# bywmm/RE-GNN

Measured on NVIDIA B200. Metric: GTEPS fwd+bwd per RE-layer, higher is better.
Workload: dtype f32

## Files before the change

re_gnn_b200/csrc/spmm.cu:

```cuda
#include <initializer_list>

#include "common.cuh"

namespace regnn {

struct SpmmArgs {
  const int32_t* indptr;
  const int32_t* indices;
  const uint8_t* etype;
  const float* theta;
  float alpha;
  int R;
  const float* norm_src;
  const float* norm_dst;
  const float* X;
  int64_t ldx;
  float* Y;
  int64_t ldy;
  int64_t row_begin, row_end;
  int F;
  const int32_t* frag_row;
  const int32_t* frag_begin;
  int nfrag, nfrag_pad, threshold;
  float* partial;
// ... 508 lines not shown
    const int64_t vi = wi * GPW + grp;
    int64_t v = -1;
    int begin = 0, len = 0;
    const bool is_frag = vi < a.nfrag;
    if (vi < nitems) {
      if (is_frag) {
        v = a.frag_row[vi];
        begin = a.frag_begin[vi];
        len = min(a.threshold, a.indptr[v + 1] - begin);
      } else {
        v = sa.order[vi - a.nfrag];
        begin = a.indptr[v];
        len = a.indptr[v + 1] - begin;
      }
    }
    const int maxlen = __reduce_max_sync(0xffffffffu, len);
    const float nd = (v >= 0 && a.norm_dst != nullptr) ? a.norm_dst[v] : 1.f;
    float4 trow = make_float4(0.f, 0.f, 0.f, 0.f);
    if (BINS && v >= 0 && col_ok) trow = ldg4(sa.Xrow + (size_t)v * sa.ldr + lg * 4);
    const bool want_ydg = DNORM && (sa.dn_sides & 2) && v >= 0 && col_ok && !is_frag;
    if constexpr (DNORM) {
      if (want_ydg) {
        prefetch_l2(sa.Yfwd + (size_t)v * sa.ldyf + lg * 4);
        prefetch_l2(xbytes + (uint64_t)(uint32_t)v * ldxb);
      }
    }
    float4 acc = make_float4(0.f, 0.f, 0.f, 0.f);
    int cur_rel = 0;
    float racc = 0.f;
    const int32_t* ip = a.indices + begin;
    const uint8_t* ep = a.etype + begin;

    if constexpr (kCoop) {
      static_assert(G % U == 0, "a round must not straddle a slot batch");
      const int gbase = lane & ~(G - 1);
      auto load_batch = [&](int t0, int& bi, int& be, float& bn) {
        const int t = t0 + lg;
        bi = -1;
        be = 0;
        bn = 0.f;
        if (t < len) {
          bi = __ldg(ip + t);
          be = weighted ? (int)__ldg(ep + t) : 0;
          bn = a.norm_src != nullptr ? __ldg(a.norm_src + bi) : 1.f;
        }
      };
      int nbi, nbe;
      float nbn;
      load_batch(0, nbi, nbe, nbn);
      for (int t0 = 0; t0 < maxlen; t0 += G) {
        const int bi = nbi, be = nbe;
        const float bn = nbn;
        const float bc = (weighted ? w_s[be] : 1.f) * bn;
        if (t0 + G < maxlen) load_batch(t0 + G, nbi, nbe, nbn);
        const int cnt = min(G, maxlen - t0);
        for (int j = 0; j < cnt; j += U) {
          float4 x[U];
#pragma unroll
          for (int u = 0; u < U; ++u) {
            const int si = __shfl_sync(0xffffffffu, bi, gbase + j + u);
            x[u] = si >= 0 ? ldg4(reinterpret_cast<const float*>(xbytes + (uint64_t)(uint32_t)si * ldxb))
                           : make_float4(0.f, 0.f, 0.f, 0.f);
          }
#pragma unroll
          for (int u = 0; u < U; ++u) {
            const int from = gbase + j + u;
            fma4(acc, __shfl_sync(0xffffffffu, bc, from), x[u]);
            if (BINS) {
              const int se = __shfl_sync(0xffffffffu, be, from);
              const float sn = __shfl_sync(0xffffffffu, bn, from);
              const float d = dot4(x[u], trow);
              if (t0 + j + u < len && se != cur_rel) {
                mybins[cur_rel * 32] += racc;
                racc = 0.f;
                cur_rel = se;
              }
              racc = fmaf(sn * nd, d, racc);
            }
          }
        }
      }
    } else {
      int nidx[U], net[U];
#pragma unroll
      for (int u = 0; u < U; ++u) {
        nidx[u] = u < len ? __ldg(ip + u) : -1;
        net[u] = (weighted && u < len) ? (int)__ldg(ep + u) : 0;
      }
      for (int t = 0; t < maxlen; t += U) {
        int idx[U], et[U];
#pragma unroll
        for (int u = 0; u < U; ++u) {
          idx[u] = nidx[u];
          et[u] = net[u];
        }
        float4 x[U];
        float ns[U];
#pragma unroll
        for (int u = 0; u < U; ++u) {
          x[u] = idx[u] >= 0 ? ldg4(reinterpret_cast<const float*>(xbytes + (uint64_t)(uint32_t)idx[u] * ldxb))
                             : make_float4(0.f, 0.f, 0.f, 0.f);
          ns[u] = idx[u] >= 0 ? (a.norm_src != nullptr ? __ldg(a.norm_src + idx[u]) : 1.f) : 0.f;
        }
#pragma unroll
        for (int u = 0; u < U; ++u) {
          const int tn = t + U + u;
          nidx[u] = tn < len ? __ldg(ip + tn) : -1;
          net[u] = (weighted && tn < len) ? (int)__ldg(ep + tn) : 0;
        }
#pragma unroll
        for (int u = 0; u < U; ++u) {
          const float coef = (weighted ? w_s[et[u]] : 1.f) * ns[u];
          fma4(acc, coef, x[u]);
          if (BINS) {
            const float d = dot4(x[u], trow);
            if (idx[u] >= 0 && et[u] != cur_rel) {
              mybins[cur_rel * 32] += racc;
              racc = 0.f;
              cur_rel = et[u];
            }
            racc = fmaf(ns[u] * nd, d, racc);
          }
        }
      }
    }
    if (BINS) {
      mybins[cur_rel * 32] += racc;
      if constexpr (DNORM) {
        float p = (sa.dn_sides & 1) ? dot4(acc, trow) * nd : 0.f;
        if (want_ydg)
          p += dot4(ldg4(sa.Yfwd + (size_t)v * sa.ldyf + lg * 4),
                    ldg4(reinterpret_cast<const float*>(xbytes + (uint64_t)(uint32_t)v * ldxb)));
        p = group_sum<G>(p);
        if (lg == 0 && v >= 0 && !is_frag) sa.d_norm[v] = p / sa.norm[v];
      } else if (sa.xdx != nullptr) {
        const float d = group_sum<G>(dot4(acc, trow)) * nd;
        if (lg == 0 && v >= 0 && !is_frag) sa.xdx[v] = d;
      }
    }
    if (v >= 0 && col_ok) {
      if (is_frag) {
        st4(a.partial + (size_t)vi * a.F + lg * 4, acc);
      } else {
        scale4(acc, nd);
        float* yrow = sa.peers.base != nullptr ? sa.peers.row(v) : a.Y + (size_t)v * a.ldy;
        st4(yrow + lg * 4, acc);
        if (!BINS && sa.peers.base != nullptr && sa.Ylocal != nullptr) st4(sa.Ylocal + (size_t)v * sa.ldl + lg * 4, acc);
      }
    }
  }
  if (BINS) reduce_bins(bins, scratch, a.R, sa.partials + (size_t)blockIdx.x * a.R);
}

constexpr int kRowdotRows = 4;
__global__ void __launch_bounds__(kWarpsPerBlock * 32)
rowdot_norm_kernel(const float* __restrict__ norm, int sides, const float* __restrict__ X, int64_t ldx,
                   const float* __restrict__ Y, int64_t ldy, const float* __restrict__ G, int64_t ldg,
                   const float* __restrict__ dX, int64_t lddx, const float* __restrict__ xdx, int F,
                   int64_t row_begin, int64_t row_end, float* __restrict__ d_norm) {
  const int lane = threadIdx.x & 31;
  const int64_t v0 = row_begin + ((int64_t)blockIdx.x * kWarpsPerBlock + (threadIdx.x >> 5)) * kRowdotRows;
  if (v0 >= row_end) return;
  const bool use_x = (sides & 1) && xdx == nullptr;
  const bool vec = (F & 3) == 0 && ((ldy | ldg) & 3) == 0 && ((((uintptr_t)Y) | ((uintptr_t)G)) & 15) == 0 &&
                   (!use_x || (((ldx | lddx) & 3) == 0 && ((((uintptr_t)X) | ((uintptr_t)dX)) & 15) == 0));
  float p[kRowdotRows];
#pragma unroll
  for (int r = 0; r < kRowdotRows; ++r) p[r] = 0.f;
  if (vec) {
    for (int c = lane * 4; c < F; c += 128) {
#pragma unroll
      for (int r = 0; r < kRowdotRows; ++r) {
        const int64_t v = v0 + r;
        if (v < row_end) {
          if (sides & 2) p[r] += dot4(ldg4(Y + (size_t)v * ldy + c), ldg4(G + (size_t)v * ldg + c));
          if (use_x) p[r] += dot4(ldg4(X + (size_t)v * ldx + c), ldg4(dX + (size_t)v * lddx + c));
        }
      }
    }
  } else {
    for (int c = lane; c < F; c += 32) {
#pragma unroll
      for (int r = 0; r < kRowdotRows; ++r) {
        const int64_t v = v0 + r;
        if (v < row_end) {
          if (sides & 2) p[r] = fmaf(__ldg(Y + (size_t)v * ldy + c), __ldg(G + (size_t)v * ldg + c), p[r]);
          if (use_x) p[r] = fmaf(__ldg(X + (size_t)v * ldx + c), __ldg(dX + (size_t)v * lddx + c), p[r]);
        }
      }
    }
  }
#pragma unroll
  for (int r = 0; r < kRowdotRows; ++r) {
    const int64_t v = v0 + r;
    float t = group_sum<32>(p[r]);
    if (v < row_end && lane == 0) {
      if ((sides & 1) && xdx != nullptr) t += xdx[v];
      d_norm[v] = t / norm[v];
    }
  }
}

__global__ void long_row_dnorm_kernel(const int32_t* __restrict__ long_rows, int num_long, const float* __restrict__ X,
                                      int64_t ldx, const float* __restrict__ dX, int64_t lddx, int F, int64_t row_begin,
                                      int64_t row_end, float* __restrict__ xdx, const float* __restrict__ Y, int64_t ldy,
                                      const float* __restrict__ Gd, int64_t ldg, const float* __restrict__ norm, int sides,
                                      float* __restrict__ d_norm) {
  const int lane = threadIdx.x & 31;
  const int l = blockIdx.x * (blockDim.x >> 5) + (threadIdx.x >> 5);
  if (l >= num_long) return;
  const int64_t v = long_rows[l];
  if (v < row_begin || v >= row_end) return;
  float p = 0.f, q = 0.f;
  if (xdx != nullptr || (sides & 1))
    for (int c = lane; c < F; c += 32) p = fmaf(__ldg(X + (size_t)v * ldx + c), dX[(size_t)v * lddx + c], p);
  if (d_norm != nullptr && (sides & 2))
    for (int c = lane; c < F; c += 32) q = fmaf(__ldg(Y + (size_t)v * ldy + c), __ldg(Gd + (size_t)v * ldg + c), q);
  p = group_sum<32>(p);
  q = group_sum<32>(q);
  if (lane == 0) {
    if (xdx != nullptr) xdx[v] = p;
    if (d_norm != nullptr) d_norm[v] = (((sides & 1) ? p : 0.f) + q) / norm[v];
  }
}

struct SpmmBwdArgs {
  const int32_t* indptr;
  const int32_t* indices;
  const uint8_t* etype;
  int R;
  const float* norm;
  int sides;
  const float* X;  int64_t ldx;
  const float* Y;  int64_t ldy;
  const float* G;  int64_t ldg;
  const float* dX; int64_t lddx;
  int64_t row_begin, row_end;
  int F;
  double* partials;
  float* d_norm;
  const int32_t* frag_row;
  const int32_t* frag_begin;
  int nfrag, threshold;
};

template <int G, int C, int VW, bool WEIGHTED>
__global__ void __launch_bounds__(kWarpsPerBlock * 32)
spmm_bwd_w_kernel(SpmmBwdArgs a) {
  using V = Vec<VW>;
  using T = typename V::T;
  constexpr int U = Unroll<C>::U;
  constexpr int GPW = 32 / G;
  extern __shared__ __align__(16) unsigned char smem_raw[];
  double* scratch = reinterpret_cast<double*>(smem_raw);
  float* bins = reinterpret_cast<float*>(scratch + kWarpsPerBlock * a.R);
  const int lane = threadIdx.x & 31, warp = threadIdx.x >> 5;
  const int lg = lane % G, grp = lane / G;
  float* mybins = bins + (size_t)warp * a.R * 32 + lane;
  if (WEIGHTED)
    for (int r = 0; r < a.R; ++r) mybins[r * 32] = 0.f;

  bool col_ok[C];
#pragma unroll
  for (int k = 0; k < C; ++k) col_ok[k] = (lg + k * G) * VW < a.F;
  const int64_t rows = a.row_end - a.row_begin;
  const int64_t nfrag_groups = (a.nfrag + GPW - 1) / GPW;
  const int64_t ngroups = nfrag_groups + (rows + GPW - 1) / GPW;

  for (int64_t rg = (int64_t)blockIdx.x * kWarpsPerBlock + warp; rg < ngroups;
       rg += (int64_t)gridDim.x * kWarpsPerBlock) {
    bool row_ok = false, first = true;
    int64_t v = 0;
    int s0 = 0, len = 0;
    if (rg < nfrag_groups) {
      const int64_t fi = rg * GPW + grp;
      if (fi < a.nfrag) {
        v = a.frag_row[fi];
        if (v >= a.row_begin && v < a.row_end) {
          s0 = a.frag_begin[fi];
          len = min(a.threshold, a.indptr[v + 1] - s0);
          first = s0 == a.indptr[v];
          row_ok = true;
        }
      }
    } else {
      v = a.row_begin + (rg - nfrag_groups) * GPW + grp;
      if (v < a.row_end) {
        s0 = a.indptr[v];
        len = a.indptr[v + 1] - s0;
        row_ok = len <= a.threshold;
        if (!row_ok) len = 0;
      }
    }
    float nv = 1.f;
    T g[C];
    float p = 0.f;
    if (row_ok) nv = a.norm != nullptr ? a.norm[v] : 1.f;
#pragma unroll
    for (int k = 0; k < C; ++k) {
      g[k] = V::zero();
      if (row_ok && col_ok[k]) {
        const size_t c = (size_t)(lg + k * G) * VW;
        g[k] = V::load(a.G + (size_t)v * a.ldg + c);
        if (first && a.d_norm != nullptr) {
          if (a.sides & 2) p += V::dot(V::load(a.Y + (size_t)v * a.ldy + c), g[k]);
          if (a.sides & 1) p += V::dot(V::load(a.X + (size_t)v * a.ldx + c), V::load(a.dX + (size_t)v * a.lddx + c));
// ... 281 lines not shown

#define REGNN_DISPATCH_GC(G_, C_, VW_, CALL)                    \
  if (sh.G == G_ && sh.C == C_ && sh.VW == VW_) {               \
    constexpr int G = G_, C = C_, VW = VW_;                     \
    CALL;                                                       \
    launched = true;                                            \
  }
#define REGNN_DISPATCH_SHAPES(CALL)                                                            \
  REGNN_DISPATCH_GC(4, 1, 4, CALL) REGNN_DISPATCH_GC(8, 1, 4, CALL) REGNN_DISPATCH_GC(16, 1, 4, CALL) \
  REGNN_DISPATCH_GC(16, 2, 4, CALL) REGNN_DISPATCH_GC(16, 3, 4, CALL)                          \
  REGNN_DISPATCH_GC(32, 1, 4, CALL) REGNN_DISPATCH_GC(32, 2, 4, CALL) REGNN_DISPATCH_GC(32, 3, 4, CALL) \
  REGNN_DISPATCH_GC(32, 4, 4, CALL) REGNN_DISPATCH_GC(32, 8, 4, CALL)                          \
  REGNN_DISPATCH_GC(4, 1, 1, CALL) REGNN_DISPATCH_GC(8, 1, 1, CALL) REGNN_DISPATCH_GC(16, 1, 1, CALL) \
  REGNN_DISPATCH_GC(32, 1, 1, CALL) REGNN_DISPATCH_GC(32, 2, 1, CALL) REGNN_DISPATCH_GC(32, 3, 1, CALL) \
  REGNN_DISPATCH_GC(32, 4, 1, CALL) REGNN_DISPATCH_GC(32, 8, 1, CALL)

}

using namespace regnn;

extern "C" int regnn_relation_counts(const int32_t* row, const uint8_t* etype_csr, int64_t num_edges,
                                     int64_t num_nodes, int num_relations, int32_t* counts, void* stream) {
  REGNN_REQUIRE(counts && (num_edges == 0 || (row && etype_csr)), REGNN_ERR_INVALID_ARG, "relation_counts: null pointer");
  REGNN_REQUIRE(num_relations >= 1 && num_relations <= REGNN_MAX_RELATIONS, REGNN_ERR_UNSUPPORTED_SHAPE,
                "num_relations=%d outside [1,%d]", num_relations, REGNN_MAX_RELATIONS);
  cudaMemsetAsync(counts, 0, (size_t)num_nodes * num_relations * sizeof(int32_t), (cudaStream_t)stream);
  if (num_edges > 0)
    relation_count_kernel<<<(unsigned)((num_edges + 255) / 256), 256, 0, (cudaStream_t)stream>>>(row, etype_csr, num_edges,
                                                                                               num_relations, counts);
  return check_launch("regnn_relation_counts");
}

extern "C" int regnn_wdeg_norm_fwd(const int32_t* indptr, const uint8_t* etype_csr, const int32_t* counts,
                                   const float* theta, float alpha, int num_relations,
                                   float exponent, float clamp_min, int64_t row_begin, int64_t row_end, float* deg,
                                   float* norm, void* stream) {
  REGNN_REQUIRE(theta && norm && (counts || (indptr && etype_csr)), REGNN_ERR_INVALID_ARG, "wdeg_norm_fwd: null pointer");
  REGNN_REQUIRE(num_relations >= 1 && num_relations <= REGNN_MAX_RELATIONS, REGNN_ERR_UNSUPPORTED_SHAPE,
                "num_relations=%d outside [1,%d]", num_relations, REGNN_MAX_RELATIONS);
  const int64_t rows = row_end - row_begin;
  REGNN_REQUIRE(rows >= 0, REGNN_ERR_INVALID_ARG, "wdeg_norm_fwd: empty/negative row range");
  if (rows == 0) return REGNN_OK;
  const int threads = kWarpsPerBlock * 32;
  if (counts != nullptr) {
    wdeg_norm_fwd_cnt_kernel<<<(unsigned)((rows + threads - 1) / threads), threads, 0, (cudaStream_t)stream>>>(
        counts, theta, alpha, num_relations, exponent, clamp_min, row_begin, row_end, deg, norm);
  } else if (num_relations <= 32) {
    const int64_t blocks = (rows + kWarpsPerBlock * kWdegRows - 1) / (kWarpsPerBlock * kWdegRows);
    wdeg_norm_fwd_slot_kernel<<<(unsigned)blocks, threads, 0, (cudaStream_t)stream>>>(
        indptr, etype_csr, theta, alpha, num_relations, exponent, clamp_min, row_begin, row_end, deg, norm);
  } else {
    const int64_t blocks = (rows * 8 + threads - 1) / threads;
    wdeg_norm_fwd_kernel<<<(unsigned)blocks, threads, 0, (cudaStream_t)stream>>>(
        indptr, etype_csr, theta, alpha, num_relations, exponent, clamp_min, row_begin, row_end, deg, norm);
  }
  return check_launch("regnn_wdeg_norm_fwd");
}

static size_t bins_smem_bytes(int R) { return (size_t)kWarpsPerBlock * R * (sizeof(double) + 32 * sizeof(float)); }

extern "C" int regnn_wdeg_norm_bwd(const int32_t* indptr, const uint8_t* etype_csr, const int32_t* counts,
                                   const float* theta, float alpha, int num_relations,
                                   float exponent, float clamp_min, int64_t row_begin, int64_t row_end,
                                   const float* deg, const float* d_norm, double* partials,
                                   float* d_theta, void* stream_) {
  cudaStream_t stream = (cudaStream_t)stream_;
  REGNN_REQUIRE((counts || (indptr && etype_csr)) && theta && deg && d_norm && partials && d_theta,
                REGNN_ERR_INVALID_ARG, "wdeg_norm_bwd: null pointer");
  const int R = num_relations;
  REGNN_REQUIRE(R >= 1 && R <= REGNN_MAX_RELATIONS, REGNN_ERR_UNSUPPORTED_SHAPE, "num_relations=%d outside [1,%d]", R,
                REGNN_MAX_RELATIONS);
  const int64_t rows = row_end - row_begin;
  REGNN_REQUIRE(rows >= 0, REGNN_ERR_INVALID_ARG, "wdeg_norm_bwd: negative row range");
  const int nb = partial_blocks(rows);
  const size_t smem = bins_smem_bytes(R);
  int rc = REGNN_OK;
  if (counts != nullptr) {
    if ((rc = set_smem(wdeg_norm_bwd_cnt_kernel, smem)) != REGNN_OK) return rc;
    wdeg_norm_bwd_cnt_kernel<<<nb, kWarpsPerBlock * 32, smem, stream>>>(counts, R, exponent, clamp_min, row_begin, row_end, deg,
                                                                         d_norm, partials);
  } else if (R <= 32) {
    if ((rc = set_smem(wdeg_norm_bwd_slot_kernel, smem)) != REGNN_OK) return rc;
    wdeg_norm_bwd_slot_kernel<<<nb, kWarpsPerBlock * 32, smem, stream>>>(indptr, etype_csr, R, exponent, clamp_min, row_begin,
                                                                          row_end, deg, d_norm, partials);
  } else {
    if ((rc = set_smem(wdeg_norm_bwd_kernel, smem)) != REGNN_OK) return rc;
    wdeg_norm_bwd_kernel<<<nb, kWarpsPerBlock * 32, smem, stream>>>(indptr, etype_csr, R, exponent, clamp_min,
                                                                     row_begin, row_end, deg, d_norm, partials);
  }
  launch_relation_grad_finalize(partials, nb, R, R, theta, alpha, d_theta, stream);
  return check_launch("regnn_wdeg_norm_bwd");
}

struct StreamShape { int C, VW; };

static bool aligned_to(const void* p, int bytes) { return ((uintptr_t)p & (bytes - 1)) == 0; }

static bool pick_stream_shape(int F, int align, StreamShape* sh) {
  int VW = 1;
  if (align >= 16 && F % 4 == 0 && F >= 96) VW = 4;
  else if (align >= 8 && F % 2 == 0 && F >= 34) VW = 2;
  int C = (F + 32 * VW - 1) / (32 * VW);
  if (C > 8) {
    if (VW == 1 && align >= 8 && F % 2 == 0) { VW = 2; C = (F + 63) / 64; }
    if (C > 8 && align >= 16 && F % 4 == 0) { VW = 4; C = (F + 127) / 128; }
    if (C > 8) return false;
  }
  if (C > 4) C = 8;
  *sh = {C, VW};
  return true;
}

static int common_align(std::initializer_list<const void*> ptrs, std::initializer_list<int64_t> lds) {
  int al = 16;
  for (const void* p : ptrs)
    while (p != nullptr && al > 4 && !aligned_to(p, al)) al >>= 1;
  for (int64_t ld : lds)
    while (al > 4 && (ld * 4) % al != 0) al >>= 1;
  return al;
}

#define REGNN_STREAM_CASE(C_, VW_, BINS_, CALL)     \
  if (sh.C == C_ && sh.VW == VW_) {                 \
    constexpr int C = C_, VW = VW_;                 \
    constexpr bool BINS = BINS_;                    \
    CALL;                                           \
    launched = true;                                \
  }
#define REGNN_STREAM_DISPATCH(BINS_, CALL)                                                          \
  REGNN_STREAM_CASE(1, 4, BINS_, CALL) REGNN_STREAM_CASE(2, 4, BINS_, CALL) REGNN_STREAM_CASE(3, 4, BINS_, CALL) \
  REGNN_STREAM_CASE(4, 4, BINS_, CALL) REGNN_STREAM_CASE(8, 4, BINS_, CALL)                          \
  REGNN_STREAM_CASE(1, 2, BINS_, CALL) REGNN_STREAM_CASE(2, 2, BINS_, CALL) REGNN_STREAM_CASE(3, 2, BINS_, CALL) \
  REGNN_STREAM_CASE(4, 2, BINS_, CALL) REGNN_STREAM_CASE(8, 2, BINS_, CALL)                          \
  REGNN_STREAM_CASE(1, 1, BINS_, CALL) REGNN_STREAM_CASE(2, 1, BINS_, CALL) REGNN_STREAM_CASE(3, 1, BINS_, CALL) \
  REGNN_STREAM_CASE(4, 1, BINS_, CALL) REGNN_STREAM_CASE(8, 1, BINS_, CALL)

#ifndef REGNN_RG_MAXF
#define REGNN_RG_MAXF 128
#endif
static int rowgroup_lanes(int F, const int32_t* order, int64_t row_begin, int align) {
  if (order == nullptr || row_begin != 0 || F > REGNN_RG_MAXF || F % 4 != 0 || align < 16) return 0;
  return F > 64 ? 32 : (F > 32 ? 16 : (F > 16 ? 8 : 4));
}
#define REGNN_ROWGROUP_CASE(G_, BINS_, CALL) \
  if (G == G_) {                             \
    constexpr int GL = G_;                   \
    constexpr bool BINS = BINS_;             \
    CALL;                                    \
    launched = true;                         \
  }
#define REGNN_ROWGROUP_DISPATCH(BINS_, CALL)                                                               \
  REGNN_ROWGROUP_CASE(32, BINS_, CALL) REGNN_ROWGROUP_CASE(16, BINS_, CALL) REGNN_ROWGROUP_CASE(8, BINS_, CALL) \
  REGNN_ROWGROUP_CASE(4, BINS_, CALL)


static int fill_split(SpmmArgs& a, const regnn_rowsplit_t* split, float* ws, const char* who) {
  a.frag_row = a.frag_begin = nullptr;
  a.nfrag = a.nfrag_pad = 0;
  a.threshold = 0x7fffffff;
  a.partial = ws;
  if (split == nullptr || split->num_frags <= 0) return REGNN_OK;
  REGNN_REQUIRE(ws && split->long_rows && split->frag_ptr && split->frag_row && split->frag_begin && split->threshold > 0,
                REGNN_ERR_INVALID_ARG, "%s: incomplete row split", who);
  a.frag_row = split->frag_row;
  a.frag_begin = split->frag_begin;
  a.nfrag = split->num_frags;
  a.nfrag_pad = (a.nfrag + kWarpsPerBlock - 1) / kWarpsPerBlock * kWarpsPerBlock;
  a.threshold = split->threshold;
  return REGNN_OK;
}

static int fill_peers(PeerRows* out, const regnn_peer_rows_t* peers, int feat, int64_t rows, const char* who) {
  *out = PeerRows{nullptr, 1u, 0, 0};
  if (peers == nullptr) return REGNN_OK;
  REGNN_REQUIRE(peers->base != nullptr && peers->num_ranks >= 1 && peers->rows_per_rank >= 1 &&
                    peers->rows_per_rank < (1ll << 31) && rows <= peers->rows_per_rank * peers->num_ranks &&
                    peers->col_offset >= 0 && peers->col_offset % 4 == 0 && peers->ld % 4 == 0 &&
                    peers->ld >= peers->col_offset + feat,
                REGNN_ERR_INVALID_ARG, "%s: bad peer row-block table", who);
  *out = PeerRows{peers->base, (uint32_t)peers->rows_per_rank, peers->ld, peers->col_offset};
  return REGNN_OK;
}

static int spmm_fwd_impl(const int32_t* indptr, const int32_t* indices, const uint8_t* etype,
                         const float* theta, float alpha, int num_relations,
                         const float* norm_src, const float* norm_dst, const float* X,
                         int64_t ldx, float* Y, int64_t ldy, int64_t row_begin,
                         int64_t row_end, int feat, const regnn_rowsplit_t* split,
                         float* split_workspace, const int32_t* row_order, const regnn_peer_rows_t* peers,
                         float* y_local, int64_t ldl, void* stream_) {
  cudaStream_t stream = (cudaStream_t)stream_;
  if (peers != nullptr) { Y = const_cast<float*>(X); ldy = feat; }
  REGNN_REQUIRE(y_local == nullptr || (peers != nullptr && ldl >= feat && ldl % 4 == 0 && aligned_to(y_local, 16)),
                REGNN_ERR_INVALID_ARG, "spmm_fwd: bad local result slab");
  REGNN_REQUIRE(indptr && X && Y,   REGNN_ERR_INVALID_ARG, "spmm_fwd: null pointer");
  REGNN_REQUIRE(etype == nullptr || theta != nullptr, REGNN_ERR_INVALID_ARG, "spmm_fwd: etype without theta");
  REGNN_REQUIRE(etype == nullptr || (num_relations >= 1 && num_relations <= REGNN_MAX_RELATIONS),
                REGNN_ERR_UNSUPPORTED_SHAPE, "num_relations=%d outside [1,%d]", num_relations, REGNN_MAX_RELATIONS);
  REGNN_REQUIRE(feat >= 1 && ldx >= feat && ldy >= feat, REGNN_ERR_INVALID_ARG, "spmm_fwd: bad feature width / leading dimension");
  const int64_t rows = row_end - row_begin;
  REGNN_REQUIRE(rows >= 0, REGNN_ERR_INVALID_ARG, "spmm_fwd: negative row range");
  if (rows == 0) return REGNN_OK;
  StreamShape sh;
  REGNN_REQUIRE(pick_stream_shape(feat, common_align({X, Y, split_workspace}, {ldx, ldy, (int64_t)feat}), &sh),
                REGNN_ERR_UNSUPPORTED_SHAPE, "spmm_fwd: feature width %d too wide (max 1024 aligned / 256 unaligned)", feat);
  StreamArgs sa{};
  sa.s = SpmmArgs{indptr, indices, etype, theta, alpha, num_relations, norm_src, norm_dst, X, ldx, Y, ldy,
                  row_begin, row_end, feat, nullptr, nullptr, 0, 0, 0x7fffffff, nullptr};
  int rc = fill_split(sa.s, split, split_workspace, "spmm_fwd");
  if (rc != REGNN_OK) return rc;
  bool launched = false;
  const int G = rowgroup_lanes(feat, row_order, row_begin, common_align({X, Y, split_workspace}, {ldx, ldy, (int64_t)feat}));
  rc = fill_peers(&sa.peers, peers, feat, rows, "spmm_fwd");
  if (rc != REGNN_OK) return rc;
  sa.Ylocal = y_local;
  sa.ldl = ldl;
  REGNN_REQUIRE(peers == nullptr || G != 0, REGNN_ERR_UNSUPPORTED_SHAPE,
                "spmm_fwd: the peer scatter needs the lane-group kernel (row_order, full range, F <= 128, F %% 4 == 0)");
  if (G != 0) {
    REGNN_REQUIRE(ldx < (1ll << 30), REGNN_ERR_UNSUPPORTED_SHAPE, "spmm_fwd: leading dimension too large");
    sa.order = row_order;
    sa.n_order = rows - (sa.s.nfrag > 0 ? split->num_long : 0);
    const int64_t nwork = (sa.s.nfrag + sa.n_order + 32 / G - 1) / (32 / G);
    const unsigned blocks = (unsigned)((nwork + kWarpsPerBlock - 1) / kWarpsPerBlock);
    REGNN_ROWGROUP_DISPATCH(false, (spmm_rowgroup_kernel<BINS, GL><<<blocks, kWarpsPerBlock * 32, 0, stream>>>(sa)))
  } else {
    const int64_t nitems = sa.s.nfrag_pad + (rows + kRowsPerItem - 1) / kRowsPerItem;
    const unsigned blocks = (unsigned)((nitems + kWarpsPerBlock - 1) / kWarpsPerBlock);
    REGNN_STREAM_DISPATCH(false, (spmm_stream_kernel<C, VW, BINS><<<blocks, kWarpsPerBlock * 32, 0, stream>>>(sa)))
  }
  REGNN_REQUIRE(launched, REGNN_ERR_UNSUPPORTED_SHAPE, "spmm_fwd: no kernel for C=%d VW=%d", sh.C, sh.VW);
  if (sa.s.nfrag > 0 && peers != nullptr)
    spmm_frag_finalize_peer_kernel<<<split->num_long, 128, 0, stream>>>(
        split->long_rows, split->frag_ptr, split->num_long, split_workspace, norm_dst, sa.peers, feat,
        FragPeerExtra{y_local, ldl, nullptr, 0, nullptr, nullptr, 0, nullptr, 0, nullptr, 0, nullptr});
  else if (sa.s.nfrag > 0)
    spmm_frag_finalize_kernel<<<split->num_long, 128, 0, stream>>>(split->long_rows, split->frag_ptr, split->num_long,
                                                                   split_workspace, norm_dst, Y, ldy, feat, row_begin, row_end);
  return check_launch("regnn_spmm_fwd");
}

extern "C" int regnn_spmm_fwd(const int32_t* indptr, const int32_t* indices, const uint8_t* etype,
                              const float* theta, float alpha, int num_relations,
                              const float* norm_src, const float* norm_dst, const float* X,
                              int64_t ldx, float* Y, int64_t ldy, int64_t row_begin,
                              int64_t row_end, int feat, const regnn_rowsplit_t* split,
                              float* split_workspace, const int32_t* row_order, void* stream) {
  return spmm_fwd_impl(indptr, indices, etype, theta, alpha, num_relations, norm_src, norm_dst, X, ldx, Y, ldy,
                       row_begin, row_end, feat, split, split_workspace, row_order, nullptr, nullptr, 0, stream);
}

extern "C" int regnn_spmm_fwd_scatter(const int32_t* indptr, const int32_t* indices, const uint8_t* etype,
                                      const float* theta, float alpha, int num_relations,
                                      const float* norm_src, const float* norm_dst, const float* X,
                                      int64_t ldx, int64_t num_rows, int feat, const regnn_rowsplit_t* split,
                                      float* split_workspace, const int32_t* row_order,
                                      const regnn_peer_rows_t* peers, float* y_local, int64_t ldl, void* stream) {
  REGNN_REQUIRE(peers != nullptr, REGNN_ERR_INVALID_ARG, "spmm_fwd_scatter: null peer table");
  return spmm_fwd_impl(indptr, indices, etype, theta, alpha, num_relations, norm_src, norm_dst, X, ldx, nullptr, 0,
                       0, num_rows, feat, split, split_workspace, row_order, peers, y_local, ldl, stream);
}

extern "C" int regnn_rows_to_slabs(const float* X, int64_t ldx, int64_t num_rows, int feat, int num_ranks,
                                   int64_t row_offset, float* const* peer_slabs, void* stream) {
  REGNN_REQUIRE(X && peer_slabs && num_ranks >= 1 && num_rows >= 0 && row_offset >= 0, REGNN_ERR_INVALID_ARG,
                "rows_to_slabs: bad argument");
  REGNN_REQUIRE(feat % (4 * num_ranks) == 0 && ldx % 4 == 0 && aligned_to(X, 16), REGNN_ERR_UNSUPPORTED_SHAPE,
                "rows_to_slabs: F=%d must split into whole 128-bit chunks over %d ranks (16-byte aligned rows)", feat,
                num_ranks);
  if (num_rows == 0) return REGNN_OK;
  const int Fc = feat / num_ranks;
  const int64_t total = num_rows * (Fc / 4);
  const int64_t want = (total + 255) / 256;
  const unsigned bx = (unsigned)(want < 148 * 8 ? want : 148 * 8);
  const int first_peer = (int)((row_offset / (num_rows > 0 ? num_rows : 1)) % num_ranks);
  rows_to_slabs_kernel<<<dim3(bx, (unsigned)num_ranks), 256, 0, (cudaStream_t)stream>>>(X, ldx, num_rows, Fc, row_offset,
                                                                                     peer_slabs, first_peer);
  return check_launch("regnn_rows_to_slabs");
}

extern "C" int regnn_halo_push(const float* X, int64_t ldx, int feat, const int32_t* send_rows, const int64_t* send_ptr,
                               const int64_t* recv_offset, float* const* peer_bufs, int64_t ldb, int num_ranks, int rank,
                               void* stream) {
  REGNN_REQUIRE(X && send_ptr && recv_offset && peer_bufs && num_ranks >= 1 && rank >= 0 && rank < num_ranks,
                REGNN_ERR_INVALID_ARG, "halo_push: bad argument");
  REGNN_REQUIRE(num_ranks <= REGNN_HALO_MAX_RANKS, REGNN_ERR_UNSUPPORTED_SHAPE, "halo_push: %d ranks (max %d)", num_ranks,
                REGNN_HALO_MAX_RANKS);
  REGNN_REQUIRE(feat >= 4 && feat % 4 == 0 && ldx >= feat && ldb >= feat && ldx % 4 == 0 && ldb % 4 == 0 &&
                    aligned_to(X, 16),
                REGNN_ERR_UNSUPPORTED_SHAPE, "halo_push: F=%d must be whole 128-bit chunks in 16-byte aligned rows", feat);
  HaloPeers hp;
  int64_t most = 0;
  hp.ptr[0] = send_ptr[0];
  REGNN_REQUIRE(send_ptr[0] >= 0, REGNN_ERR_INVALID_ARG, "halo_push: negative send offset");
  for (int q = 0; q < num_ranks; ++q) {
    const int64_t cnt = send_ptr[q + 1] - send_ptr[q];
    REGNN_REQUIRE(cnt >= 0 && recv_offset[q] >= 0, REGNN_ERR_INVALID_ARG,
                  "halo_push: peer %d has a negative row count or receive offset", q);
    hp.ptr[q + 1] = send_ptr[q + 1];
    hp.recv_offset[q] = recv_offset[q];
    most = cnt > most ? cnt : most;
  }
  if (most == 0) return REGNN_OK;
  REGNN_REQUIRE(send_rows != nullptr, REGNN_ERR_INVALID_ARG, "halo_push: null send list");
  const int L = feat / 4;
  int G = 1;
  while (G < L && G < 32) G <<= 1;
  const int64_t want = (most * G + 255) / 256;
  const unsigned bx = (unsigned)(want < 148 * 8 ? want : 148 * 8);
  halo_push_kernel<<<dim3(bx, (unsigned)num_ranks), 256, 0, (cudaStream_t)stream>>>(X, ldx, L, G, send_rows, hp,
                                                                                  peer_bufs, ldb, rank);
  return check_launch("regnn_halo_push");
}

extern "C" int regnn_halo_scatter(const float* X, int64_t ldx, int width, const int64_t* send_ptr, const int32_t* dst_rows,
                                  float* const* peer_bufs, int64_t ldb, int num_ranks, int rank, void* stream) {
  REGNN_REQUIRE(X && send_ptr && peer_bufs && num_ranks >= 1 && rank >= 0 && rank < num_ranks, REGNN_ERR_INVALID_ARG,
                "halo_scatter: bad argument");
  REGNN_REQUIRE(num_ranks <= REGNN_HALO_MAX_RANKS, REGNN_ERR_UNSUPPORTED_SHAPE, "halo_scatter: %d ranks (max %d)",
                num_ranks, REGNN_HALO_MAX_RANKS);
  REGNN_REQUIRE(width >= 1 && ldx >= width && ldb >= width, REGNN_ERR_INVALID_ARG,
                "halo_scatter: W=%d with leading dimensions %lld / %lld", width, (long long)ldx, (long long)ldb);
  REGNN_REQUIRE(send_ptr[0] >= 0, REGNN_ERR_INVALID_ARG, "halo_scatter: negative send offset");
  HaloPeers hp;
  int64_t most = 0;
  hp.ptr[0] = send_ptr[0];
  for (int q = 0; q < num_ranks; ++q) {
    const int64_t cnt = send_ptr[q + 1] - send_ptr[q];
    REGNN_REQUIRE(cnt >= 0, REGNN_ERR_INVALID_ARG, "halo_scatter: peer %d has a negative row count", q);
    hp.ptr[q + 1] = send_ptr[q + 1];
    hp.recv_offset[q] = 0;
    most = cnt > most ? cnt : most;
  }
  if (most == 0) return REGNN_OK;
  REGNN_REQUIRE(dst_rows != nullptr, REGNN_ERR_INVALID_ARG, "halo_scatter: null destination rows");
  const int64_t want = (most * width + 255) / 256;
  const unsigned bx = (unsigned)(want < 148 * 8 ? want : 148 * 8);
  halo_scatter_kernel<<<dim3(bx, (unsigned)num_ranks), 256, 0, (cudaStream_t)stream>>>(X, ldx, width, dst_rows, hp,
                                                                                     peer_bufs, ldb, rank);
  return check_launch("regnn_halo_scatter");
}

extern "C" int regnn_slabs_to_rows(const float* S, int64_t lds, int64_t num_rows, int feat,
                                   const regnn_peer_rows_t* peers, void* stream) {
  REGNN_REQUIRE(S && peers && num_rows >= 0 && feat >= 4 && feat % 4 == 0 && lds % 4 == 0 && aligned_to(S, 16),
                REGNN_ERR_INVALID_ARG, "slabs_to_rows: bad argument (16-byte aligned rows of whole 128-bit chunks)");
  PeerRows pr;
  int rc = fill_peers(&pr, peers, feat, num_rows, "slabs_to_rows");
  if (rc != REGNN_OK) return rc;
  if (num_rows == 0) return REGNN_OK;
  const int64_t total = (int64_t)pr.per * (feat / 4);
  const int64_t want = (total + 255) / 256;
  const unsigned bx = (unsigned)(want < 148 * 8 ? want : 148 * 8);
  const int first_peer = (int)((peers->col_offset / feat) % peers->num_ranks);
  slabs_to_rows_kernel<<<dim3(bx, (unsigned)peers->num_ranks), 256, 0, (cudaStream_t)stream>>>(S, lds, num_rows, feat, pr,
                                                                                              first_peer);
  return check_launch("regnn_slabs_to_rows");
}

static int spmm_bwd_fused_impl(const int32_t* indptr_t, const int32_t* indices_t,
                               const uint8_t* etype_t, const float* theta, float alpha,
                               int num_relations, const float* norm, int norm_sides, const float* X,
                               int64_t ldx, const float* Gd, int64_t ldg, float* dX, int64_t lddx,
                               int64_t row_begin, int64_t row_end, int feat, double* partials,
                               float* d_theta, float* xdx, const float* Yfwd, int64_t ldyf, float* d_norm,
                               const regnn_rowsplit_t* split_t,
                               float* split_workspace, const int32_t* row_order_t, const regnn_peer_rows_t* peers,
                               void* stream_) {
  cudaStream_t stream = (cudaStream_t)stream_;
  if (peers != nullptr) { dX = const_cast<float*>(X); lddx = ldx; }
  REGNN_REQUIRE(indptr_t && theta && X && Gd && dX && partials && d_theta,
                REGNN_ERR_INVALID_ARG, "spmm_bwd_fused: null pointer");
  const int R = num_relations;
  REGNN_REQUIRE(R >= 1 && R <= REGNN_MAX_RELATIONS, REGNN_ERR_UNSUPPORTED_SHAPE, "num_relations=%d outside [1,%d]", R,
                REGNN_MAX_RELATIONS);
  REGNN_REQUIRE(feat >= 1 && ldx >= feat && ldg >= feat && lddx >= feat, REGNN_ERR_INVALID_ARG,
                "spmm_bwd_fused: bad feature width / leading dimension");
  const int64_t rows = row_end - row_begin;
  REGNN_REQUIRE(rows >= 0, REGNN_ERR_INVALID_ARG, "spmm_bwd_fused: negative row range");
  StreamShape sh;
  REGNN_REQUIRE(pick_stream_shape(feat, common_align({X, Gd, dX, split_workspace}, {ldx, ldg, lddx, (int64_t)feat}), &sh),
                REGNN_ERR_UNSUPPORTED_SHAPE, "spmm_bwd_fused: feature width %d too wide", feat);
  const int sides = norm != nullptr ? (norm_sides & 3) : 0;
  StreamArgs sa{};
  sa.s = SpmmArgs{indptr_t, indices_t, etype_t, theta, alpha, R, (sides & 2) ? norm : nullptr, (sides & 1) ? norm : nullptr,
                  Gd, ldg, dX, lddx, row_begin, row_end, feat, nullptr, nullptr, 0, 0, 0x7fffffff, nullptr};
  int rc = fill_split(sa.s, split_t, split_workspace, "spmm_bwd_fused");
  if (rc != REGNN_OK) return rc;
  sa.Xrow = X;
  sa.ldr = ldx;
  sa.partials = partials;
  sa.use_tma = (feat % 4 == 0 && aligned_to(X, 16) && ldx % 4 == 0) ? 1 : 0;
  sa.xdx = xdx;
  const int Fp = (feat + 3) & ~3;
  if (d_norm != nullptr) {
    REGNN_REQUIRE(norm != nullptr && (!(sides & 2) || (Yfwd != nullptr && ldyf >= feat)),
                  REGNN_ERR_INVALID_ARG, "spmm_bwd_fused: d_norm needs norm and (destination side scaled) Y");
    REGNN_REQUIRE(!(sides & 2) || (aligned_to(Yfwd, 16) && ldyf % 4 == 0), REGNN_ERR_INVALID_ARG,
                  "spmm_bwd_fused: Y rows must be 16-byte aligned");
    sa.Yfwd = Yfwd; sa.ldyf = ldyf; sa.norm = norm; sa.dn_sides = sides; sa.d_norm = d_norm;
  }
  const size_t smem = 64 + (size_t)kWarpsPerBlock * R * (sizeof(double) + 32 * sizeof(float)) +
                      (size_t)kWarpsPerBlock * kRowsPerItemBins * Fp * sizeof(float);
  int nb = partial_blocks(rows / kRowsPerItemBins + sa.s.nfrag + 1);
  bool launched = false;
  const int G = rowgroup_lanes(feat, row_order_t, row_begin,
                               common_align({X, Gd, dX, split_workspace}, {ldx, ldg, lddx, (int64_t)feat}));
  rc = fill_peers(&sa.peers, peers, feat, rows, "spmm_bwd_fused");
  if (rc != REGNN_OK) return rc;
  REGNN_REQUIRE(peers == nullptr || G != 0, REGNN_ERR_UNSUPPORTED_SHAPE,
                "spmm_bwd_fused: the peer scatter needs the lane-group kernel (row_order_t, full range, F <= 128, F %% 4 == 0)");
  REGNN_REQUIRE(d_norm == nullptr || G != 0, REGNN_ERR_UNSUPPORTED_SHAPE,
                "spmm_bwd_fused: the folded norm gradient needs the lane-group kernel (row_order_t, full range, F <= 128, "
                "F %% 4 == 0); use regnn_rowdot_norm_bwd otherwise");
  if (G != 0) {
    REGNN_REQUIRE(ldg < (1ll << 30), REGNN_ERR_UNSUPPORTED_SHAPE, "spmm_bwd_fused: leading dimension too large");
    sa.order = row_order_t;
    sa.n_order = rows - (sa.s.nfrag > 0 ? split_t->num_long : 0);
    const size_t gsmem = (size_t)kWarpsPerBlock * R * (sizeof(double) + 32 * sizeof(float));
    if (d_norm != nullptr) {
      REGNN_ROWGROUP_DISPATCH(true, (rc = set_smem(spmm_rowgroup_kernel<BINS, GL, true>, gsmem),
                                     nb = min(nb, resident_blocks(spmm_rowgroup_kernel<BINS, GL, true>, gsmem)),
                                     spmm_rowgroup_kernel<BINS, GL, true><<<nb, kWarpsPerBlock * 32, gsmem, stream>>>(sa)))
    } else {
      REGNN_ROWGROUP_DISPATCH(true, (rc = set_smem(spmm_rowgroup_kernel<BINS, GL>, gsmem),
                                     nb = min(nb, resident_blocks(spmm_rowgroup_kernel<BINS, GL>, gsmem)),
                                     spmm_rowgroup_kernel<BINS, GL><<<nb, kWarpsPerBlock * 32, gsmem, stream>>>(sa)))
    }
  } else {
    REGNN_STREAM_DISPATCH(true, (rc = set_smem(spmm_stream_kernel<C, VW, BINS>, smem),
                                 nb = min(nb, resident_blocks(spmm_stream_kernel<C, VW, BINS>, smem)),
                                 spmm_stream_kernel<C, VW, BINS><<<nb, kWarpsPerBlock * 32, smem, stream>>>(sa)))
  }
  if (rc != REGNN_OK) return rc;
  REGNN_REQUIRE(launched, REGNN_ERR_UNSUPPORTED_SHAPE, "spmm_bwd_fused: no kernel for C=%d VW=%d", sh.C, sh.VW);
  if (sa.s.nfrag > 0 && peers != nullptr)
    spmm_frag_finalize_peer_kernel<<<split_t->num_long, 128, 0, stream>>>(
        split_t->long_rows, split_t->frag_ptr, split_t->num_long, split_workspace, sa.s.norm_dst, sa.peers, feat,
        FragPeerExtra{nullptr, 0, X, ldx, xdx, Yfwd, ldyf, Gd, ldg, norm, sides, d_norm});
  else if (sa.s.nfrag > 0)
    spmm_frag_finalize_kernel<<<split_t->num_long, 128, 0, stream>>>(split_t->long_rows, split_t->frag_ptr,
                                                                     split_t->num_long, split_workspace, sa.s.norm_dst, dX,
                                                                     lddx, feat, row_begin, row_end);
  if (sa.s.nfrag > 0 && (xdx != nullptr || d_norm != nullptr) && peers == nullptr)
    long_row_dnorm_kernel<<<(split_t->num_long + 3) / 4, 128, 0, stream>>>(split_t->long_rows, split_t->num_long, X, ldx, dX,
                                                                           lddx, feat, row_begin, row_end, xdx, Yfwd, ldyf, Gd,
                                                                           ldg, norm, sides, d_norm);
  launch_relation_grad_finalize(partials, nb, R, R, theta, alpha, d_theta, stream);
  return check_launch("regnn_spmm_bwd_fused");
}

extern "C" int regnn_spmm_bwd_fused(const int32_t* indptr_t, const int32_t* indices_t,
                                    const uint8_t* etype_t, const float* theta, float alpha,
                                    int num_relations, const float* norm, int norm_sides, const float* X,
                                    int64_t ldx, const float* Gd, int64_t ldg, float* dX, int64_t lddx,
                                    int64_t row_begin, int64_t row_end, int feat, double* partials,
                                    float* d_theta, float* xdx, const float* Y, int64_t ldy, float* d_norm,
                                    const regnn_rowsplit_t* split_t,
                                    float* split_workspace, const int32_t* row_order_t, void* stream) {
  return spmm_bwd_fused_impl(indptr_t, indices_t, etype_t, theta, alpha, num_relations, norm, norm_sides, X, ldx, Gd, ldg,
                             dX, lddx, row_begin, row_end, feat, partials, d_theta, xdx, Y, ldy, d_norm, split_t,
                             split_workspace, row_order_t, nullptr, stream);
}

extern "C" int regnn_spmm_bwd_fused_scatter(const int32_t* indptr_t, const int32_t* indices_t,
                                            const uint8_t* etype_t, const float* theta, float alpha,
                                            int num_relations, const float* norm, int norm_sides, const float* X,
                                            int64_t ldx, const float* Gd, int64_t ldg, int64_t num_rows, int feat,
                                            double* partials, float* d_theta, float* xdx, const float* Y, int64_t ldy,
                                            float* d_norm, const regnn_rowsplit_t* split_t, float* split_workspace,
                                            const int32_t* row_order_t, const regnn_peer_rows_t* peers, void* stream) {
  REGNN_REQUIRE(peers != nullptr, REGNN_ERR_INVALID_ARG, "spmm_bwd_fused_scatter: null peer table");
  return spmm_bwd_fused_impl(indptr_t, indices_t, etype_t, theta, alpha, num_relations, norm, norm_sides, X, ldx, Gd, ldg,
                             nullptr, 0, 0, num_rows, feat, partials, d_theta, xdx, Y, ldy, d_norm, split_t,
                             split_workspace, row_order_t, peers, stream);
}

extern "C" int regnn_rowdot_norm_bwd(const float* norm, int norm_sides, const float* X, int64_t ldx,
                                     const float* Y, int64_t ldy, const float* Gd, int64_t ldg,
                                     const float* dX, int64_t lddx, const float* xdx, int64_t row_begin,
                                     int64_t row_end, int feat, float* d_norm, void* stream) {
  REGNN_REQUIRE(norm && Y && Gd && d_norm && (xdx || (X && dX)), REGNN_ERR_INVALID_ARG, "rowdot_norm_bwd: null pointer");
  const int64_t rows = row_end - row_begin;
  REGNN_REQUIRE(rows >= 0 && feat >= 1, REGNN_ERR_INVALID_ARG, "rowdot_norm_bwd: bad range / width");
  if (rows == 0) return REGNN_OK;
  const int64_t rows_per_block = (int64_t)kWarpsPerBlock * kRowdotRows;
  rowdot_norm_kernel<<<(unsigned)((rows + rows_per_block - 1) / rows_per_block), kWarpsPerBlock * 32, 0,
                       (cudaStream_t)stream>>>(norm, norm_sides & 3, X, ldx, Y, ldy, Gd, ldg, dX, lddx, xdx, feat,
                                               row_begin, row_end, d_norm);
  return check_launch("regnn_rowdot_norm_bwd");
}

extern "C" int regnn_spmm_bwd_w(const int32_t* indptr, const int32_t* indices, const uint8_t* etype,
                                const float* theta, float alpha, int num_relations,
                                const float* norm, int norm_sides, const float* X, int64_t ldx, const float* Y,
                                int64_t ldy, const float* Gd, int64_t ldg, const float* dX,
                                int64_t lddx, int64_t row_begin, int64_t row_end, int feat,
                                double* partials, float* d_theta, float* d_norm,
                                const regnn_rowsplit_t* split, void* stream_) {
  cudaStream_t stream = (cudaStream_t)stream_;
  REGNN_REQUIRE(indptr && X && Y && Gd && dX, REGNN_ERR_INVALID_ARG, "spmm_bwd_w: null pointer");
  const bool weighted = etype != nullptr;
  const int R = weighted ? num_relations : 1;
  REGNN_REQUIRE(!weighted || (theta && partials && d_theta), REGNN_ERR_INVALID_ARG, "spmm_bwd_w: null relation buffers");
  REGNN_REQUIRE(R >= 1 && R <= REGNN_MAX_RELATIONS, REGNN_ERR_UNSUPPORTED_SHAPE, "num_relations=%d outside [1,%d]", R,
                REGNN_MAX_RELATIONS);
  REGNN_REQUIRE(feat >= 1 && ldx >= feat && ldy >= feat && ldg >= feat && lddx >= feat, REGNN_ERR_INVALID_ARG,
                "spmm_bwd_w: bad feature width / leading dimension");
  const int64_t rows = row_end - row_begin;
  REGNN_REQUIRE(rows >= 0, REGNN_ERR_INVALID_ARG, "spmm_bwd_w: negative row range");
  const bool vec_ok = aligned16(X) && aligned16(Y) && aligned16(Gd) && aligned16(dX) && ldx % 4 == 0 &&
                      ldy % 4 == 0 && ldg % 4 == 0 && lddx % 4 == 0;
  Shape sh;
  REGNN_REQUIRE(pick_shape(feat, vec_ok, &sh), REGNN_ERR_UNSUPPORTED_SHAPE,
                "spmm_bwd_w: feature width %d too wide", feat);
  const bool use_split = split != nullptr && split->num_frags > 0;
  REGNN_REQUIRE(!use_split || (split->frag_row && split->frag_begin && split->threshold > 0), REGNN_ERR_INVALID_ARG,
                "spmm_bwd_w: incomplete row split");
  SpmmBwdArgs a{indptr, indices, etype, R, norm, norm != nullptr ? (norm_sides & 3) : 0, X, ldx, Y, ldy, Gd, ldg, dX, lddx, row_begin, row_end,
                feat, partials, d_norm, use_split ? split->frag_row : nullptr, use_split ? split->frag_begin : nullptr,
                use_split ? split->num_frags : 0, use_split ? split->threshold : 0x7fffffff};
  const int nb = partial_blocks(rows);
  const size_t smem = weighted ? bins_smem_bytes(R) : 16;
  bool launched = false;
  int rc = REGNN_OK;
  if (weighted) {
    REGNN_DISPATCH_SHAPES((rc = set_smem(spmm_bwd_w_kernel<G, C, VW, true>, smem),
                           spmm_bwd_w_kernel<G, C, VW, true><<<nb, kWarpsPerBlock * 32, smem, stream>>>(a)))
  } else {
    REGNN_DISPATCH_SHAPES((spmm_bwd_w_kernel<G, C, VW, false><<<nb, kWarpsPerBlock * 32, smem, stream>>>(a)))
  }
  if (rc != REGNN_OK) return rc;
  REGNN_REQUIRE(launched, REGNN_ERR_UNSUPPORTED_SHAPE, "spmm_bwd_w: no kernel for G=%d C=%d VW=%d", sh.G, sh.C, sh.VW);
  if (weighted) launch_relation_grad_finalize(partials, nb, R, R, theta, alpha, d_theta, stream);
  return check_launch("regnn_spmm_bwd_w");
}
```

Baseline: 4.936.

## Add cp.async ring-buffered SpMM kernel for full-warp feature rows

```diff
diff --git a/re_gnn_b200/csrc/spmm.cu b/re_gnn_b200/csrc/spmm.cu
--- a/re_gnn_b200/csrc/spmm.cu
+++ b/re_gnn_b200/csrc/spmm.cu
@@ -684,6 +684,261 @@
   if (BINS) reduce_bins(bins, scratch, a.R, sa.partials + (size_t)blockIdx.x * a.R);
 }
 
+#ifndef REGNN_SPMM_RING
+#define REGNN_SPMM_RING 1
+#endif
+#ifndef REGNN_RING_B
+#define REGNN_RING_B 16
+#endif
+#ifndef REGNN_RING_S
+#define REGNN_RING_S 3
+#endif
+#ifndef REGNN_RING_BLOCKS
+#define REGNN_RING_BLOCKS 1
+#endif
+constexpr int kRingB = REGNN_RING_B, kRingS = REGNN_RING_S;
+constexpr int kRingPitch = 128;
+constexpr size_t kRingWarpBytes = ((size_t)kRingS * kRingB * kRingPitch * 4 + (size_t)kRingS * kRingB * 8 + kRingS * 16 +
+                                   (size_t)kRingS * 32 * 16 + kRingS * 8 + 127) & ~(size_t)127;
+static_assert(kRingB >= 1 && kRingB <= 32 && kRingS >= 2 && kRingS <= 8, "B <= 32 rows per stage, 2..8 stages");
+static_assert((kRingS * kRingB) % 2 == 0, "the int4 stage descriptors and headers must stay 16-byte aligned");
+
+__device__ __forceinline__ void cp_async16(uint32_t dst, const void* src) {
+  asm volatile("cp.async.cg.shared.global [%0], [%1], 16;" ::"r"(dst), "l"(src) : "memory");
+}
+__device__ __forceinline__ void cp_async4(uint32_t dst, const void* src) {
+  asm volatile("cp.async.ca.shared.global [%0], [%1], 4;" ::"r"(dst), "l"(src) : "memory");
+}
+__device__ __forceinline__ void cp_async_arrive_noinc(uint64_t* bar) {
+  asm volatile("cp.async.mbarrier.arrive.noinc.shared::cta.b64 [%0];" ::"r"(smem_u32(bar)) : "memory");
+}
+
+template <bool BINS, bool DNORM = false>
+__global__ void __launch_bounds__(kWarpsPerBlock * 32, REGNN_RING_BLOCKS)
+spmm_ring_kernel(StreamArgs sa) {
+  static_assert(BINS || !DNORM, "the folded norm gradient belongs to the backward kernel");
+  constexpr int B = kRingB, S = kRingS;
+  const SpmmArgs& a = sa.s;
+  __shared__ float w_s[256];
+  extern __shared__ __align__(16) unsigned char dsm[];
+  const int lane = threadIdx.x & 31, warp = threadIdx.x >> 5;
+  double* scratch = reinterpret_cast<double*>(dsm);
+  float* bins = reinterpret_cast<float*>(scratch + kWarpsPerBlock * a.R);
+  float* mybins = bins + (size_t)warp * a.R * 32 + lane;
+  unsigned char* wbase = dsm + (BINS ? (size_t)kWarpsPerBlock * a.R * (sizeof(double) + 32 * sizeof(float)) : 0) +
+                         (size_t)warp * kRingWarpBytes;
+  float* ring = reinterpret_cast<float*>(wbase);
+  float* ns_s = ring + (size_t)S * B * kRingPitch;
+  int* et_s = reinterpret_cast<int*>(ns_s + S * B);
+  int4* desc = reinterpret_cast<int4*>(et_s + S * B);
+  int4* hdr = desc + S;
+  uint64_t* bars = reinterpret_cast<uint64_t*>(hdr + S * 32);
+  const bool weighted = a.etype != nullptr;
+  if (weighted)
+    for (int i = threadIdx.x; i < a.R; i += blockDim.x) w_s[i] = leaky(a.theta[i] * a.alpha, kRelationSlope);
+  if (BINS)
+    for (int r = 0; r < a.R; ++r) mybins[r * 32] = 0.f;
+  if (lane < S) mbar_init(bars + lane, 32);
+  asm volatile("fence.mbarrier_init.release.cluster;" ::: "memory");
+  __syncthreads();
+
+  const bool col_ok = lane * 4 < a.F;
+  const char* xbytes = reinterpret_cast<const char*>(a.X + (col_ok ? lane : 0) * 4);
+  const uint32_t ldxb = (uint32_t)a.ldx * 4u;
+  const int64_t nitems = (int64_t)a.nfrag + sa.n_order;
+  const int64_t nwarps = (int64_t)gridDim.x * kWarpsPerBlock;
+  const int64_t gw = (int64_t)blockIdx.x * kWarpsPerBlock + warp;
+  const bool want_y = DNORM && (sa.dn_sides & 2);
+
+  int pbseq = -1, pcount = 0, ptotal = 0, pp = 0;
+  int pbegin = 0, pexcl = 0, pincl = 0, pv = 0;
+  bool pfirst = false, pmore = true, pfrag = false;
+  int nidx = -1, net = 0;
+  int nprod = 0;
+
+  auto decode_batch = [&]() {
+    ++pbseq;
+    const int64_t item = gw + ((int64_t)pbseq * 32 + lane) * nwarps;
+    int v = 0, begin = 0, len = 0;
+    float nd = 1.f;
+    const bool valid = item < nitems;
+    pfrag = item < a.nfrag;
+    if (valid) {
+      if (pfrag) {
+        v = a.frag_row[item];
+        begin = a.frag_begin[item];
+        len = min(a.threshold, a.indptr[v + 1] - begin);
+      } else {
+        v = sa.order[item - a.nfrag];
+        begin = a.indptr[v];
+        len = a.indptr[v + 1] - begin;
+      }
+      if (a.norm_dst != nullptr) nd = a.norm_dst[v];
+    }
+    int incl = len;
+#pragma unroll
+    for (int o = 1; o < 32; o <<= 1) {
+      const int t = __shfl_up_sync(0xffffffffu, incl, o);
+      if (lane >= o) incl += t;
+    }
+    pcount = __popc(__ballot_sync(0xffffffffu, valid));
+    ptotal = __shfl_sync(0xffffffffu, incl, 31);
+    pbegin = begin;
+    pexcl = incl - len;
+    pincl = incl;
+    pv = v;
+    if (valid) hdr[(pbseq % S) * 32 + lane] = make_int4(v, __float_as_int(nd), incl, (int)item);
+    pp = 0;
+    pfirst = true;
+  };
+  auto load_slots = [&]() {
+    const int s = pp + lane;
+    int j = 0;
+#pragma unroll
+    for (int o = 16; o > 0; o >>= 1)
+      if (__shfl_sync(0xffffffffu, pincl, j + o - 1) <= s) j += o;
+    const int jb = __shfl_sync(0xffffffffu, pbegin, j), je = __shfl_sync(0xffffffffu, pexcl, j);
+    nidx = -1;
+    net = 0;
+    if (lane < B && s < ptotal) {
+      nidx = __ldg(a.indices + jb + (s - je));
+      if (weighted) net = (int)__ldg(a.etype + jb + (s - je));
+    }
+  };
+  auto produce = [&]() {
+    if (!pmore) return;
+    if (pp >= ptotal && !pfirst) {
+      decode_batch();
+      if (pcount == 0) {
+        pmore = false;
+        return;
+      }
+      load_slots();
+    }
+    const int st = nprod % S;
+    if (BINS && lane < pcount && pexcl >= pp && (pexcl < pp + B || pp + B >= ptotal)) {
+      for (int c = 0; c < a.F; c += 32) {
+        prefetch_l2(sa.Xrow + (size_t)pv * sa.ldr + c);
+        if (want_y && !pfrag) {
+          prefetch_l2(sa.Yfwd + (size_t)pv * sa.ldyf + c);
+          prefetch_l2(a.X + (size_t)pv * a.ldx + c);
+        }
+      }
+    }
+    const uint32_t dst = smem_u32(ring + (size_t)st * B * kRingPitch + lane * 4);
+#pragma unroll
+    for (int u = 0; u < B; ++u) {
+      const int si = __shfl_sync(0xffffffffu, nidx, u);
+      if (si >= 0) cp_async16(dst + u * kRingPitch * 4, xbytes + (uint64_t)(uint32_t)si * ldxb);
+    }
+    if (nidx >= 0) {
+      if (a.norm_src != nullptr) cp_async4(smem_u32(ns_s + st * B + lane), a.norm_src + nidx);
+      else ns_s[st * B + lane] = 1.f;
+      et_s[st * B + lane] = net;
+    }
+    cp_async_arrive_noinc(bars + st);
+    if (lane == 0)
+      desc[st] = make_int4(pp, min(B, ptotal - pp), (pbseq % S) | (pfirst ? 256 : 0) | (pp + B >= ptotal ? 512 : 0),
+                           pcount);
+    pfirst = false;
+    pp += B;
+    ++nprod;
+    if (pp < ptotal) load_slots();
+  };
+
+  int cbslot = 0, ccount = 0, cj = 0, cend = 0, cv = 0, citem = 0;
+  float cnd = 1.f;
+  float4 acc = make_float4(0.f, 0.f, 0.f, 0.f), trow = acc, yv = acc, gv = acc;
+  int cur_rel = 0;
+  float racc = 0.f;
+  auto start_item = [&]() {
+    const int4 h = hdr[cbslot * 32 + cj];
+    cv = h.x;
+    cnd = __int_as_float(h.y);
+    cend = h.z;
+    citem = h.w;
+    if (BINS && col_ok) trow = ldg4(sa.Xrow + (size_t)cv * sa.ldr + lane * 4);
+    if (want_y && col_ok && citem >= a.nfrag) {
+      yv = ldg4(sa.Yfwd + (size_t)cv * sa.ldyf + lane * 4);
+      gv = ldg4(reinterpret_cast<const float*>(xbytes + (uint64_t)(uint32_t)cv * ldxb));
+    }
+  };
+  auto finish_item = [&]() {
+    const bool is_frag = citem < a.nfrag;
+    if (BINS) {
+      mybins[cur_rel * 32] += racc;
+      racc = 0.f;
+      cur_rel = 0;
+      if constexpr (DNORM) {
+        float p = (sa.dn_sides & 1) ? dot4(acc, trow) * cnd : 0.f;
+        if (want_y && !is_frag) p += dot4(yv, gv);
+        p = group_sum<32>(p);
+        if (lane == 0 && !is_frag) sa.d_norm[cv] = p / sa.norm[cv];
+      } else if (sa.xdx != nullptr) {
+        const float d = group_sum<32>(dot4(acc, trow)) * cnd;
+        if (lane == 0 && !is_frag) sa.xdx[cv] = d;
+      }
+    }
+    if (col_ok) {
+      if (is_frag) {
+        st4(a.partial + (size_t)citem * a.F + lane * 4, acc);
+      } else {
+        scale4(acc, cnd);
+        st4(a.Y + (size_t)cv * a.ldy + lane * 4, acc);
+      }
+    }
+    acc = make_float4(0.f, 0.f, 0.f, 0.f);
+  };
+
+  decode_batch();
+  if (pcount == 0) pmore = false;
+  else load_slots();
+  for (int i = 0; i < S - 1; ++i) produce();
+  for (int k = 0; k < nprod; ++k) {
+    __syncwarp();
+    produce();
+    const int st = k % S;
+    mbar_wait(bars + st, (uint32_t)(k / S) & 1u);
+    const int4 d = desc[st];
+    if (d.z & 256) {
+      cbslot = d.z & 255;
+      ccount = d.w;
+      cj = 0;
+      start_item();
+    }
+    const float* buf = ring + (size_t)st * B * kRingPitch + lane * 4;
+    const float* nss = ns_s + st * B;
+    const int* ets = et_s + st * B;
+    for (int i = 0; i < d.y; ++i) {
+      while (d.x + i >= cend) {
+        finish_item();
+        ++cj;
+        start_item();
+      }
+      const float4 x = *reinterpret_cast<const float4*>(buf + i * kRingPitch);
+      const float ns = nss[i];
+      const int se = ets[i];
+      fma4(acc, (weighted ? w_s[se] : 1.f) * ns, x);
+      if (BINS) {
+        if (se != cur_rel) {
+          mybins[cur_rel * 32] += racc;
+          racc = 0.f;
+          cur_rel = se;
+        }
+        racc = fmaf(ns * cnd, dot4(x, trow), racc);
+      }
+    }
+    if (d.z & 512) {
+      finish_item();
+      while (++cj < ccount) {
+        start_item();
+        finish_item();
+      }
+    }
+  }
+  if (BINS) reduce_bins(bins, scratch, a.R, sa.partials + (size_t)blockIdx.x * a.R);
+}
+
 constexpr int kRowdotRows = 4;
 __global__ void __launch_bounds__(kWarpsPerBlock * 32)
 rowdot_norm_kernel(const float* __restrict__ norm, int sides, const float* __restrict__ X, int64_t ldx,
@@ -1271,6 +1526,13 @@
 #define REGNN_ROWGROUP_DISPATCH(BINS_, CALL)                                                               \
   REGNN_ROWGROUP_CASE(32, BINS_, CALL) REGNN_ROWGROUP_CASE(16, BINS_, CALL) REGNN_ROWGROUP_CASE(8, BINS_, CALL) \
   REGNN_ROWGROUP_CASE(4, BINS_, CALL)
+
+static size_t ring_smem(bool bins, int R) {
+  return (bins ? bins_smem_bytes(R) : 0) + (size_t)kWarpsPerBlock * kRingWarpBytes;
+}
+static bool use_ring(int G, const regnn_peer_rows_t* peers, size_t smem) {
+  return REGNN_SPMM_RING && G == 32 && peers == nullptr && smem + 256 * sizeof(float) <= 227 * 1024;
+}
 
 
 static int fill_split(SpmmArgs& a, const regnn_rowsplit_t* split, float* ws, const char* who) {
@@ -1342,7 +1604,15 @@
     sa.n_order = rows - (sa.s.nfrag > 0 ? split->num_long : 0);
     const int64_t nwork = (sa.s.nfrag + sa.n_order + 32 / G - 1) / (32 / G);
     const unsigned blocks = (unsigned)((nwork + kWarpsPerBlock - 1) / kWarpsPerBlock);
-    REGNN_ROWGROUP_DISPATCH(false, (spmm_rowgroup_kernel<BINS, GL><<<blocks, kWarpsPerBlock * 32, 0, stream>>>(sa)))
+    const size_t rsmem = ring_smem(false, 0);
+    if (use_ring(G, peers, rsmem)) {
+      if ((rc = set_smem(spmm_ring_kernel<false>, rsmem)) != REGNN_OK) return rc;
+      const unsigned nb = (unsigned)min((int64_t)resident_blocks(spmm_ring_kernel<false>, rsmem), (int64_t)blocks);
+      spmm_ring_kernel<false><<<nb, kWarpsPerBlock * 32, rsmem, stream>>>(sa);
+      launched = true;
+    } else {
+      REGNN_ROWGROUP_DISPATCH(false, (spmm_rowgroup_kernel<BINS, GL><<<blocks, kWarpsPerBlock * 32, 0, stream>>>(sa)))
+    }
   } else {
     const int64_t nitems = sa.s.nfrag_pad + (rows + kRowsPerItem - 1) / kRowsPerItem;
     const unsigned blocks = (unsigned)((nitems + kWarpsPerBlock - 1) / kWarpsPerBlock);
@@ -1537,7 +1807,19 @@
     sa.order = row_order_t;
     sa.n_order = rows - (sa.s.nfrag > 0 ? split_t->num_long : 0);
     const size_t gsmem = (size_t)kWarpsPerBlock * R * (sizeof(double) + 32 * sizeof(float));
-    if (d_norm != nullptr) {
+    const size_t rsmem = ring_smem(true, R);
+    if (use_ring(G, peers, rsmem)) {
+      if (d_norm != nullptr) {
+        if ((rc = set_smem(spmm_ring_kernel<true, true>, rsmem)) != REGNN_OK) return rc;
+        nb = min(nb, resident_blocks(spmm_ring_kernel<true, true>, rsmem));
+        spmm_ring_kernel<true, true><<<nb, kWarpsPerBlock * 32, rsmem, stream>>>(sa);
+      } else {
+        if ((rc = set_smem(spmm_ring_kernel<true>, rsmem)) != REGNN_OK) return rc;
+        nb = min(nb, resident_blocks(spmm_ring_kernel<true>, rsmem));
+        spmm_ring_kernel<true><<<nb, kWarpsPerBlock * 32, rsmem, stream>>>(sa);
+      }
+      launched = true;
+    } else if (d_norm != nullptr) {
       REGNN_ROWGROUP_DISPATCH(true, (rc = set_smem(spmm_rowgroup_kernel<BINS, GL, true>, gsmem),
                                      nb = min(nb, resident_blocks(spmm_rowgroup_kernel<BINS, GL, true>, gsmem)),
                                      spmm_rowgroup_kernel<BINS, GL, true><<<nb, kWarpsPerBlock * 32, gsmem, stream>>>(sa)))
```

Result: slower. 2.914 (median of 6 runs) (-41.0%).
